# snphbaum/scikit-gpuppy

Hardware: AMD Instinct MI355X
Metric: GP fit+predict pts/sec (K+Cholesky, N=16384 d=8) (higher is better)
Workload: dtype f64; 1 GPU; C3: N=16384 d=8 M=16384 fit(Gram+Cholesky+alpha)+estimate_many, theta fixed; global_batch=32768, parallelism=1 GPU

## Files before the change

include/gpx.h:

```cpp
#ifndef GPX_H
#define GPX_H

#include <stdint.h>

#ifdef __cplusplus
extern "C" {
#endif

#define GPX_ABI_VERSION 1
#define GPX_MAX_D 64
#define GPX_TILE 128

#define GPX_ERR_BAD_ARG   (-1)
#define GPX_ERR_HIP       (-2)
#define GPX_ERR_NO_DEVICE (-3)
#define GPX_ERR_STATE     (-4)
#define GPX_INFO_STALLED  0x3fffffff

typedef struct gpx_handle gpx_handle;

int         gpx_abi_version(void);
const char *gpx_last_error(void);
int         gpx_device_count(void);
int         gpx_set_device(int device);
// ... 61 lines not shown
int gpx_spgp_fit(const double *x, const double *t_centered, int64_t n, int d, const double *theta, const double *xb,
                 int64_t m, gpx_spgp **out);
void gpx_spgp_free(gpx_spgp *h);
int gpx_spgp_predict(gpx_spgp *h, const double *xs, int64_t ms, double *mean , double *var );
int gpx_spgp_nll(gpx_spgp *h, double *nll);
int gpx_spgp_nll_grad(gpx_spgp *h, double *grad_out);
int gpx_spgp_dense(gpx_spgp *h, int which, double *out );
int gpx_spgp_cross(gpx_spgp *h, const double *xi, int64_t n1, const double *xj, int64_t n2, double *out );

enum {
    GPX_K_GRAM = 0,
    GPX_K_GEMM = 1,
    GPX_K_POTRF_LEAF = 2,
    GPX_K_TRSV = 3,
    GPX_K_REDUCE = 4,
    GPX_K_QUAD = 5,
    GPX_K_EXACT = 6,
    GPX_K_GEMM_SMALL = 7,
    GPX_K_TRSV_RIDE = 8,
    GPX_K_GEMM_EMU = 9,
    GPX_K_COUNT = 10
};
int gpx_profile_enable(gpx_handle *h, int level);
int gpx_profile_reset(gpx_handle *h);
int gpx_profile_read(gpx_handle *h, int kernel_class, int64_t *launches, double *total_ms, double *total_work);

int gpx_bench_mfma_f64(int iters, double *tflops);
int gpx_bench_emu_i8(int64_t rows, int64_t cols, int64_t K, int nmod, int iters, double *ms);
int gpx_emu_gemm_nt_sub(const double *A, int64_t lda, const double *B, int64_t ldb, double *C, int64_t ldc, int64_t rows, int64_t cols,
                        int64_t K);
int gpx_emu_rebuild(const int8_t *R, int64_t ldr, int64_t sr, int nmod, const int *sa, const int *sb, double *C, int64_t ldc, int64_t rows,
                    int64_t cols);
int gpx_emu_i8_gemm(const int8_t *A, const int8_t *B, int64_t rows, int64_t cols, int64_t K, int nmod, int8_t *R);
int gpx_emu_trsm_left(gpx_handle *h, double *Z, int64_t ldz, int64_t rows, const double *bound, double *Zs, int64_t tile_rows, int *status_out);
int gpx_bench_hbm(int64_t bytes, int iters, double *write_gbs, double *copy_gbs);
int gpx_bench_fp64_pipes(int blocks, int iters, int mode, double *tflops, double *cycles_per_inst, double *clock_ghz);

int gpx_dev_gram(const double *xi_dev, int64_t n1, const double *xj_dev, int64_t n2, int d, const double *theta,
                 double add_diag, int lower_only, int pad_identity,
                 double *out_dev, int64_t ld, int64_t rows_pad, int64_t cols_pad, void *stream);
int gpx_dev_gram_scaled(const double *xiw_dev, int64_t n1, const double *xjw_dev, int64_t n2, int d, double v, double add_diag,
                        int lower_only, int pad_identity, double *out_dev, int64_t ld, int64_t rows_pad, int64_t cols_pad,
                        void *stream);
int gpx_dev_gemm_nt(const double *A, int64_t lda, const double *B, int64_t ldb, double *C, int64_t ldc,
                    int64_t M, int64_t N, int64_t K, double alpha, double beta, int lower_only, void *stream);
int gpx_dev_syrk_trap(const double *A, int64_t lda, const double *B, int64_t ldb, double *C, int64_t ldc, int64_t M, int64_t off_cols,
                      int64_t K, double alpha, double beta, int *count_dev, void *stream);

enum {
    GPX_GEMM_TRI_NONE = 0,
    GPX_GEMM_TRI_A_UPPER = 1,
    GPX_GEMM_TRI_A_LOWER = 2,
    GPX_GEMM_TRI_B_LOWER = 3,
    GPX_GEMM_TRI_B_UPPER = 5
};
#define GPX_GEMM_VARIANT(wm, wn, lower, form) ((wm) | ((wn) << 4) | ((lower) << 8) | ((form) << 12))
enum { GPX_GEMM_FORM_NONE = 0, GPX_GEMM_FORM_FINE = 1, GPX_GEMM_FORM_LONGEST_FIRST = 2, GPX_GEMM_FORM_PAIRED = 3, GPX_GEMM_FORM_SMALL = 4 };
enum {
    GPX_GEMM_V_NONE = 0,
    GPX_GEMM_V_128X128 = GPX_GEMM_VARIANT(4, 4, 0, 0),
    GPX_GEMM_V_64X64 = GPX_GEMM_VARIANT(2, 2, 0, 0),
    GPX_GEMM_V_64X128 = GPX_GEMM_VARIANT(2, 4, 0, 0),
    GPX_GEMM_V_32X128 = GPX_GEMM_VARIANT(1, 4, 0, 0),
    GPX_GEMM_V_LOWER_128X128 = GPX_GEMM_VARIANT(4, 4, 1, 0),
    GPX_GEMM_V_LOWER_64X64 = GPX_GEMM_VARIANT(2, 2, 1, 0),
    GPX_GEMM_V_LOWER_32X32 = GPX_GEMM_VARIANT(1, 1, 1, 0),
// ... 46 lines not shown
```

scikit-gpuppy_amd/csrc/emu.hip:

```cpp
#include <math.h>
#include <stdint.h>
#include <stdlib.h>
#include <algorithm>

#include "common.h"

#include "gemm_tile.h"

typedef int v4i __attribute__((ext_vector_type(4)));
typedef int v16i __attribute__((ext_vector_type(16)));

constexpr int EMU_MAXL = 16;
constexpr int EMU_BT = 256;
constexpr int EMU_SLAB = 1024;
constexpr int EMU_BK = 128;

constexpr int EMU_MODULI[EMU_MAXL] = {256, 255, 253, 251, 247, 241, 239, 233, 229, 227, 223, 211, 199, 197, 193, 191};

static __constant__ const int emu_p[EMU_MAXL] = {256, 255, 253, 251, 247, 241, 239, 233, 229, 227, 223, 211, 199, 197, 193, 191};

typedef unsigned __int128 emu_u128;
struct EmuCrt {
    double m[EMU_MAXL][3], p[4], pinv;
    float c[EMU_MAXL];
    unsigned long p_lo, p_hi, half_lo, half_hi;
};
struct EmuCrtAll { EmuCrt t[EMU_MAXL + 1]; };
constexpr EmuCrtAll emu_crt_tables()
{
    EmuCrtAll all{};
    constexpr emu_u128 mask = ((emu_u128)1 << 40) - 1;
    for (int L = 2; L <= EMU_MAXL; ++L) {
        EmuCrt &t = all.t[L];
        emu_u128 P = 1;
        for (int l = 0; l < L; ++l) P *= (emu_u128)EMU_MODULI[l];
        for (int l = 0; l < L; ++l) {
            const emu_u128 M = P / (emu_u128)EMU_MODULI[l];
            const int p = EMU_MODULI[l], a = (int)(M % (emu_u128)p);
            int inv = 0;
            for (int x = 1; x < p; ++x)
                if (a * x % p == 1) { inv = x; break; }
            t.c[l] = (float)inv;
            for (int j = 0; j < 3; ++j) t.m[l][j] = (double)(unsigned long)((M >> (40 * j)) & mask);
// ... 8 lines not shown
    return all;
}
static constexpr EmuCrtAll emu_crt = emu_crt_tables();

#ifdef EMU_STAMP
constexpr int EMU_STAMP_SLOTS = 1 << 16;
__device__ unsigned long emu_stamps[EMU_STAMP_SLOTS][4];
extern "C" int gpx_emu_stamps(unsigned long *out, int n)
{
    return hipMemcpyFromSymbol(out, HIP_SYMBOL(emu_stamps), sizeof(unsigned long) * 4 * std::min(n, EMU_STAMP_SLOTS)) == hipSuccess ? 0 : GPX_ERR_HIP;
}
#endif

constexpr int EMU_NONFINITE = 0x7fffffff;

int emu_moduli()
{
    static const int v = [] { const char *e = getenv("GPX_EMU_MODULI"); const int l = e ? atoi(e) : EMU_MAXL; return std::min(EMU_MAXL, std::max(2, l)); }();
    return v;
}
bool emu_enabled(int64_t K)
{
    static const int on = [] { const char *e = getenv("GPX_EMU_F64"); return e ? atoi(e) : 1; }();
    static const long min_k = [] { const char *e = getenv("GPX_EMU_MIN_K"); return e ? atol(e) : 4096L; }();
    return on && K >= min_k && K < (1 << 17) && K % EMU_BK == 0;
}
int emu_scale_bits(int64_t K, int L)
{
    double log2p = 0.0;
    for (int l = 0; l < L; ++l) log2p += log2((double)EMU_MODULI[l]);
    return (int)floor(log2p - 1.0 - log2((double)K) - 1e-9);
}

static __device__ __forceinline__ void emu_store_residues(const double (&a)[4], int L, int8_t *__restrict__ out, long plane)
{
#pragma unroll
    for (int l = 0; l < EMU_MAXL; ++l) {
        if (l >= L) continue;
        const double p = (double)emu_p[l], pinv = 1.0 / p, h = 0.5 * p;
        unsigned packed = 0;
#pragma unroll
        for (int e = 0; e < 4; ++e) {
            double r = fma(-rint(a[e] * pinv), p, a[e]);
            r = r > h ? r - p : (r < -h ? r + p : r);
            packed |= ((unsigned)(int)r & 0xffu) << (8 * e);
        }
        *reinterpret_cast<unsigned *>(out + l * plane) = packed;
    }
}

__global__ __launch_bounds__(256) void emu_split_kernel(const double *__restrict__ X, long ldx, long rows_real, int K, int bits, int L,
                                                        int8_t *__restrict__ res, long plane, int *__restrict__ sig)
{
    const long row = blockIdx.x;
    const int t = threadIdx.x;
    __shared__ double red_max[4];
    __shared__ int red_bad[4];
    int8_t *out = res + row * (long)K;
    if (row >= rows_real) {
        for (int c = 4 * t; c < K; c += 1024)
            for (int l = 0; l < L; ++l) *reinterpret_cast<int *>(out + l * plane + c) = 0;
        if (t == 0) sig[row] = 0;
        return;
    }
    const double *x = X + row * ldx;
    double m = 0.0;
    int bad = 0;
    for (int c = 2 * t; c < K; c += 512) {
        const v2d v = *reinterpret_cast<const v2d *>(x + c);
        bad |= (int)!isfinite(v.x) | (int)!isfinite(v.y);
        m = fmax(m, fmax(fabs(v.x), fabs(v.y)));
    }
#pragma unroll
    for (int o = 32; o > 0; o >>= 1) { m = fmax(m, __shfl_xor(m, o)); bad |= __shfl_xor(bad, o); }
    if ((t & 63) == 0) { red_max[t >> 6] = m; red_bad[t >> 6] = bad; }
    __syncthreads();
    m = fmax(fmax(red_max[0], red_max[1]), fmax(red_max[2], red_max[3]));
    bad = red_bad[0] | red_bad[1] | red_bad[2] | red_bad[3];
    const int s = (bad || m == 0.0) ? 0 : bits - 1 - ilogb(m);
    if (t == 0) sig[row] = bad ? EMU_NONFINITE : s;
    for (int c = 4 * t; c < K; c += 1024) {
        const v2d v0 = *reinterpret_cast<const v2d *>(x + c), v1 = *reinterpret_cast<const v2d *>(x + c + 2);
        double a[4] = {rint(ldexp(v0.x, s)), rint(ldexp(v0.y, s)), rint(ldexp(v1.x, s)), rint(ldexp(v1.y, s))};
        if (bad) a[0] = a[1] = a[2] = a[3] = 0.0;
        emu_store_residues(a, L, out + c, plane);
    }
}

__global__ __launch_bounds__(256) void emu_split_fixed_kernel(const double *__restrict__ X, long ldx, long rows_real, int width, int bits, int L,
                                                              int8_t *__restrict__ res, long ldr, long plane, int *sig, int *status)
{
    const long row = blockIdx.x;
    const int t = threadIdx.x;
    int8_t *out = res + row * ldr;
    if (row >= rows_real) {
        for (int c = 4 * t; c < width; c += 1024)
            for (int l = 0; l < L; ++l) *reinterpret_cast<int *>(out + l * plane + c) = 0;
        return;
    }
    const double *x = X + row * ldx;
    const int s0 = sig[row];
    const bool dead = s0 == EMU_NONFINITE;
    const int s = dead ? 0 : s0;
    const double lim = ldexp(1.0, bits);
    int bad = 0, over = 0;
    for (int c = 4 * t; c < width; c += 1024) {
        const v2d v0 = *reinterpret_cast<const v2d *>(x + c), v1 = *reinterpret_cast<const v2d *>(x + c + 2);
        const double v[4] = {v0.x, v0.y, v1.x, v1.y};
        double a[4];
#pragma unroll
        for (int e = 0; e < 4; ++e) {
            a[e] = rint(ldexp(v[e], s));
            if (!isfinite(v[e])) { bad = 1; a[e] = 0.0; }
            else if (fabs(a[e]) > lim) { over = 1; a[e] = 0.0; }
            if (dead) a[e] = 0.0;
        }
        emu_store_residues(a, L, out + c, plane);
    }
    bad = __syncthreads_or(bad);
    over = __syncthreads_or(over);
    if (t == 0) {
        if (bad) sig[row] = EMU_NONFINITE;
        else if (over && !dead) atomicMax(status, 1);
    }
}

constexpr int EMU_ZERO_BOUND_SCALE = 1000;
__global__ __launch_bounds__(256) void emu_scale_from_bound_kernel(const double *__restrict__ bound, long rows, long rows_pad, int bits,
                                                                   int *__restrict__ sig, int *status)
{
    const long i = (long)blockIdx.x * 256 + threadIdx.x;
    if (i >= rows_pad) return;
    const double b = i < rows ? bound[i] : 0.0;
    int s = 0;
    if (!(b >= 0.0) || isinf(b)) atomicMax(status, 1);
    else s = b == 0.0 ? EMU_ZERO_BOUND_SCALE : bits - 2 - ilogb(b);
    sig[i] = s;
}

__global__ __launch_bounds__(512, 1) void emu_i8_gemm_kernel(const int8_t *__restrict__ A, const int8_t *__restrict__ B, long sa, long sb, int K,
                                                             int8_t *__restrict__ R, long ldr, long sr, int tm, int tn, int lda)
{
    __shared__ __attribute__((aligned(1024))) int8_t smem[2 * 2 * EMU_BT * EMU_BK];
    constexpr int STAGE = 2 * EMU_BT * EMU_BK;
    const int nwg = gridDim.x, orig = blockIdx.x;
    const int lid = xcd_chunk_start(nwg, orig & 7) + (orig >> 3);
    const int per = tm * tn, z = lid / per;
    int rem = lid - z * per;
    const int g = rem / (8 * tn), first = 8 * g, grows = std::min(8, tm - first);
    rem -= g * 8 * tn;
    const int bx = rem / grows, by = first + rem - bx * grows;

    const int t = threadIdx.x;
    const int wave = __builtin_amdgcn_readfirstlane(t >> 6), lane = t & 63;
    const int wr = wave >> 2, wc = wave & 3;
    const int drow = lane >> 3;
// ... 109 lines not shown
#pragma unroll
    for (int l = 0; l < EMU_MAXL; ++l)
        w[l] = l < L ? *reinterpret_cast<const unsigned *>(R + l * sr + i * ldr + j0) : 0u;
    const int si = sa[i];
    double *c = C + i * ldc + j0;
    const __int128 P = (__int128)(((emu_u128)T.p_hi << 64) | T.p_lo), half = (__int128)(((emu_u128)T.half_hi << 64) | T.half_lo);
#pragma unroll
    for (int e = 0; e < 4; ++e) {
        if (j0 + e >= cols) continue;
        const int tj = sb[j0 + e];
        if (si == EMU_NONFINITE || tj == EMU_NONFINITE) { c[e] = __builtin_nan(""); continue; }
        double s0 = 0.0, s1 = 0.0, s2 = 0.0;
#pragma unroll
        for (int l = 0; l < EMU_MAXL; ++l) {
            const float pl = (float)emu_p[l], plinv = 1.0f / pl;
            float t = (float)(int8_t)(w[l] >> (8 * e)) * T.c[l];
            t = fmaf(-rintf(t * plinv), pl, t);
            const double td = (double)t;
            s0 = fma(td, T.m[l][0], s0);
            s1 = fma(td, T.m[l][1], s1);
            s2 = fma(td, T.m[l][2], s2);
        }
        const double q = rint(fma(fma(s2, 0x1p40, s1), 0x1p40, s0) * T.pinv);
        const long x0 = (long)fma(-q, T.p[0], s0), x1 = (long)fma(-q, T.p[1], s1), x2 = (long)fma(-q, T.p[2], s2), x3 = (long)(-q * T.p[3]);
        __int128 X = (__int128)((emu_u128)(__int128)x0 + ((emu_u128)(__int128)x1 << 40) + ((emu_u128)(__int128)x2 << 80) + ((emu_u128)(__int128)x3 << 120));
        X = X >= half ? X - P : (X < -half ? X + P : X);
        const long hi = (long)(X >> 64);
        const unsigned long lo = (unsigned long)X;
        const double xd = (hi == ((long)lo >> 63)) ? (double)(long)lo : fma((double)hi, 0x1p64, (double)lo);
        c[e] -= ldexp(xd, -(si + tj));
    }
}

static int64_t emu_cap(int64_t K, int L) { return std::max<int64_t>(EMU_BT, (((int64_t)1 << 31) / (K * L)) / EMU_BT * EMU_BT); }

void emu_work_need(EmuWork &w, int64_t rows, int64_t cols, int64_t K)
{
    const int L = emu_moduli();
    const int64_t cap = emu_cap(K, L), rt = std::min(round_up(rows, EMU_BT), cap), ct = std::min(round_up(cols, EMU_BT), cap);
    w.a_bytes = std::max(w.a_bytes, rt * K * L);
    w.b_bytes = std::max(w.b_bytes, ct * K * L);
    w.r_bytes = std::max(w.r_bytes, std::min(rt * ct * L, (int64_t)1 << 31));
    w.sig_n = std::max(w.sig_n, rt + ct);
}

int emu_work_alloc(EmuWork &w, Scratch &sc)
{
    GPX_TRY(sc.take(&w.ra, w.a_bytes));
    GPX_TRY(sc.take(&w.rb, w.b_bytes));
    GPX_TRY(sc.take(&w.rr, w.r_bytes));
    return sc.take(&w.sig, w.sig_n);
}

static int emu_check_args(const double *A, int64_t lda, const double *B, int64_t ldb, int64_t ldc, int64_t cols, int64_t K)
{
    if (K <= 0 || K % EMU_BK || K >= (1 << 17)) {
        gpx_set_error("emu_gemm_nt_sub: K = %ld is not a multiple of %d in [%d, 2^17)", (long)K, EMU_BK, EMU_BK);
        return GPX_ERR_BAD_ARG;
    }
    if (lda < K || ldb < K || ldc < cols) {
        gpx_set_error("emu_gemm_nt_sub: leading dimension shorter than a row (lda %ld, ldb %ld < K %ld, or ldc %ld < cols %ld)", (long)lda, (long)ldb,
                      (long)K, (long)ldc, (long)cols);
        return GPX_ERR_BAD_ARG;
    }
    if ((lda | ldb) & 1 || ((uintptr_t)A | (uintptr_t)B) & 15) {
        gpx_set_error("emu_gemm_nt_sub: A and B must be 16-byte aligned with even lda, ldb (lda %ld, ldb %ld, A %p, B %p)", (long)lda, (long)ldb,
                      (const void *)A, (const void *)B);
        return GPX_ERR_BAD_ARG;
    }
    return 0;
}

int emu_gemm_nt_sub(const double *A, int64_t lda, const double *B, int64_t ldb, double *C, int64_t ldc, int64_t rows, int64_t cols, int64_t K,
                    const EmuWork &w, hipStream_t s, Profiler *prof)
{
    if (rows <= 0 || cols <= 0) return 0;
    if (K % EMU_BK || K >= (1 << 17)) { gpx_set_error("emu_gemm_nt_sub: K = %ld out of range", (long)K); return GPX_ERR_BAD_ARG; }
    const int L = emu_moduli();
    const int bits = emu_scale_bits(K, L), abits = bits - bits / 2, bbits = bits / 2;
    const int64_t cap = emu_cap(K, L);
    const int64_t rt = std::min<int64_t>(round_up(rows, EMU_BT), cap);
    int64_t ct = std::min<int64_t>(round_up(cols, EMU_BT), cap);
    while (ct > EMU_BT && rt * ct * L > ((int64_t)1 << 31)) ct -= EMU_BT;
    if (!w.ra || rt * K * L > w.a_bytes || ct * K * L > w.b_bytes || rt * ct * L > w.r_bytes || rt + ct > w.sig_n) {
        gpx_set_error("emu_gemm_nt_sub: workspace too small for %ld x %ld x %ld", (long)rows, (long)cols, (long)K);
        return GPX_ERR_STATE;
    }
    ProfScope ps(prof, s, GPX_K_GEMM_EMU, 2.0 * (double)rows * (double)cols * (double)K);
    int8_t *ra = w.ra, *rb = w.rb, *rr = w.rr;
    int *sga = w.sig, *sgb = sga + rt;
    for (int64_t r0 = 0; r0 < rows; r0 += rt) {
        const int64_t nr = std::min(rt, rows - r0), nrp = round_up(nr, EMU_BT);
        hipLaunchKernelGGL(emu_split_kernel, dim3((unsigned)nrp), dim3(256), 0, s, A + r0 * lda, (long)lda, (long)nr, (int)K, abits, L, ra,
                           (long)(nrp * K), sga);
        for (int64_t c0 = 0; c0 < cols; c0 += ct) {
            const int64_t nc = std::min(ct, cols - c0), ncp = round_up(nc, EMU_BT);
            hipLaunchKernelGGL(emu_split_kernel, dim3((unsigned)ncp), dim3(256), 0, s, B + c0 * ldb, (long)ldb, (long)nc, (int)K, bbits, L, rb,
                               (long)(ncp * K), sgb);
            const int tm = (int)(nrp / EMU_BT), tn = (int)(ncp / EMU_BT);
            hipLaunchKernelGGL(emu_i8_gemm_kernel, dim3((unsigned)(tm * tn * L)), dim3(512), 0, s, (const int8_t *)ra, (const int8_t *)rb,
                               (long)(nrp * K), (long)(ncp * K), (int)K, rr, (long)ncp, (long)(nrp * ncp), tm, tn, (int)K);
            const long thr = (long)nr * ((nc + 3) / 4);
            hipLaunchKernelGGL(emu_rebuild_kernel, dim3((unsigned)((thr + 255) / 256)), dim3(256), 0, s, (const int8_t *)rr, (long)ncp,
                               (long)(nrp * ncp), L, emu_crt.t[L], (const int *)sga, (const int *)sgb, C + r0 * ldc + c0, (long)ldc, (long)nr, (long)nc);
        }
        GPX_HIP(hipGetLastError());
    }
    return 0;
}

bool emu_left_enabled()
{
    static const int on = [] { const char *e = getenv("GPX_EMU_LEFT"); return e ? atoi(e) : 1; }();
    return on != 0;
}

bool emu_left_route(bool bounded, bool few, bool ready, int64_t slabs)
{
    return bounded && !few && ready && slabs >= 5 && emu_left_enabled() && emu_enabled(4 * EMU_SLAB);
}

void emu_left_plan(EmuLeft &w, int64_t rows, int64_t slabs, int64_t tile_rows)
{
    w.L = emu_moduli();
    w.lda = EMU_SLAB * (slabs - 1);
    const int bits = emu_scale_bits(w.lda, w.L);
    w.abits = bits - bits / 2;
    w.bbits = bits / 2;
    w.rows_pad = round_up(rows, EMU_BT);
    int64_t cap = emu_cap(w.lda, w.L);
    if (tile_rows > 0) cap = std::min(cap, round_up(tile_rows, EMU_BT));
// ... 5 lines not shown
}

int emu_left_alloc(EmuLeft &w, Scratch &sc)
{
    int rc = sc.take(&w.img, w.img_bytes);
    if (!rc) rc = sc.take(&w.rb, w.b_bytes);
    if (!rc) rc = sc.take(&w.rr, w.r_bytes);
    if (!rc) rc = sc.take(&w.sig, w.rows_pad + EMU_SLAB + 1);
    if (!rc) rc = sc.take(&w.bound, w.rows_pad);
    if (rc) {
        for (void *p : {(void *)w.img, (void *)w.rb, (void *)w.rr, (void *)w.sig, (void *)w.bound})
            if (p) dfree(sc.release((double *)p));
        w.img = w.rb = w.rr = nullptr;
        w.sig = nullptr;
        w.bound = nullptr;
    }
    return rc;
}

int emu_left_begin(const EmuLeft &w, const double *bound, int64_t rows, hipStream_t s)
{
    if (rows > w.rows_pad) { gpx_set_error("emu_left_begin: %ld rows in a workspace of %ld", (long)rows, (long)w.rows_pad); return GPX_ERR_STATE; }
    GPX_HIP(hipMemsetAsync(w.status(), 0, sizeof(int), s));
    hipLaunchKernelGGL(emu_scale_from_bound_kernel, dim3((unsigned)((w.rows_pad + 255) / 256)), dim3(256), 0, s, bound, (long)rows, (long)w.rows_pad,
                       w.abits, w.sig, w.status());
    GPX_HIP(hipGetLastError());
    return 0;
}

int emu_left_split(const EmuLeft &w, const double *X, int64_t ldx, int64_t rows, int64_t q, hipStream_t s)
{
    for (int64_t t = 0, r0 = 0; r0 < rows; ++t, r0 += w.rt) {
        const int64_t nr = std::min(w.rt, rows - r0), nrp = round_up(nr, EMU_BT);
        hipLaunchKernelGGL(emu_split_fixed_kernel, dim3((unsigned)nrp), dim3(256), 0, s, X + r0 * ldx, (long)ldx, (long)nr, EMU_SLAB, w.abits, w.L,
                           w.img + t * w.rt * w.lda * w.L + q * EMU_SLAB, (long)w.lda, (long)(w.rt * w.lda), w.sig + r0, w.status());
    }
    GPX_HIP(hipGetLastError());
    return 0;
}

int emu_left_update(const EmuLeft &w, const double *B, int64_t ldb, double *C, int64_t ldc, int64_t rows, int64_t cols, int64_t K, hipStream_t s,
                    Profiler *prof)
{
    if (K <= 0 || K > w.lda || K % EMU_SLAB || cols <= 0 || cols > EMU_SLAB || rows > w.rows_pad) {
        gpx_set_error("emu_left_update: %ld x %ld x %ld outside the image", (long)rows, (long)cols, (long)K);
        return GPX_ERR_STATE;
    }
    ProfScope ps(prof, s, GPX_K_GEMM_EMU, 2.0 * (double)rows * (double)cols * (double)K);
    const int64_t ncp = round_up(cols, EMU_BT);
    int *sgb = w.sig + w.rows_pad;
    hipLaunchKernelGGL(emu_split_kernel, dim3((unsigned)ncp), dim3(256), 0, s, B, (long)ldb, (long)cols, (int)K, w.bbits, w.L, w.rb, (long)(ncp * K), sgb);
    for (int64_t t = 0, r0 = 0; r0 < rows; ++t, r0 += w.rt) {
        const int64_t nr = std::min(w.rt, rows - r0), nrp = round_up(nr, EMU_BT);
        const int tm = (int)(nrp / EMU_BT), tn = (int)(ncp / EMU_BT);
        hipLaunchKernelGGL(emu_i8_gemm_kernel, dim3((unsigned)(tm * tn * w.L)), dim3(512), 0, s, (const int8_t *)(w.img + t * w.rt * w.lda * w.L),
                           (const int8_t *)w.rb, (long)(w.rt * w.lda), (long)(ncp * K), (int)K, w.rr, (long)ncp, (long)(nrp * ncp), tm, tn, (int)w.lda);
        const long thr = (long)nr * ((cols + 3) / 4);
        hipLaunchKernelGGL(emu_rebuild_kernel, dim3((unsigned)((thr + 255) / 256)), dim3(256), 0, s, (const int8_t *)w.rr, (long)ncp, (long)(nrp * ncp), w.L,
                           emu_crt.t[w.L], (const int *)(w.sig + r0), (const int *)sgb, C + r0 * ldc, (long)ldc, (long)nr, (long)cols);
    }
    GPX_HIP(hipGetLastError());
    return 0;
}

extern "C" int gpx_emu_gemm_nt_sub(const double *A, int64_t lda, const double *B, int64_t ldb, double *C, int64_t ldc, int64_t rows, int64_t cols,
                                   int64_t K)
{
    GPX_TRY(gpx_require_device());
    if (rows < 0 || cols < 0 || !A || !B || !C) { gpx_set_error("gpx_emu_gemm_nt_sub: bad arguments"); return GPX_ERR_BAD_ARG; }
    GPX_TRY(emu_check_args(A, lda, B, ldb, ldc, cols, K));
    if (rows == 0 || cols == 0) return 0;
    Scratch sc(0);
    EmuWork w;
    emu_work_need(w, rows, cols, K);
    GPX_TRY(emu_work_alloc(w, sc));
    int rc = emu_gemm_nt_sub(A, lda, B, ldb, C, ldc, rows, cols, K, w, 0, nullptr);
    if (hipStreamSynchronize(0) != hipSuccess && rc == 0) { gpx_set_error("gpx_emu_gemm_nt_sub: stream failed"); rc = GPX_ERR_HIP; }
    return rc;
}

extern "C" int gpx_emu_rebuild(const int8_t *R, int64_t ldr, int64_t sr, int nmod, const int *sa, const int *sb, double *C, int64_t ldc, int64_t rows,
                               int64_t cols)
{
    GPX_TRY(gpx_require_device());
    if (!R || !sa || !sb || !C || rows < 0 || cols < 0 || nmod < 2 || nmod > EMU_MAXL || ldr < round_up(cols, 4) || (ldr | sr) & 3 ||
        (uintptr_t)R & 3 || sr < rows * ldr || ldc < cols) {
        gpx_set_error("gpx_emu_rebuild: bad arguments");
        return GPX_ERR_BAD_ARG;
    }
    if (rows == 0 || cols == 0) return 0;
    const long thr = (long)rows * ((cols + 3) / 4);
    hipLaunchKernelGGL(emu_rebuild_kernel, dim3((unsigned)((thr + 255) / 256)), dim3(256), 0, 0, R, (long)ldr, (long)sr, nmod, emu_crt.t[nmod], sa, sb, C,
                       (long)ldc, (long)rows, (long)cols);
    GPX_HIP(hipGetLastError());
    GPX_HIP(hipStreamSynchronize(0));
    return 0;
}

extern "C" int gpx_emu_i8_gemm(const int8_t *A, const int8_t *B, int64_t rows, int64_t cols, int64_t K, int nmod, int8_t *R)
{
    GPX_TRY(gpx_require_device());
    if (!A || !B || !R || rows <= 0 || cols <= 0 || rows % EMU_BT || cols % EMU_BT || K <= 0 || K % EMU_BK || K >= (1 << 17) || nmod < 1 ||
        nmod > EMU_MAXL || ((uintptr_t)A | (uintptr_t)B) & 15 || rows / EMU_BT * (cols / EMU_BT) * nmod > INT32_MAX) {
        gpx_set_error("gpx_emu_i8_gemm: bad arguments");
        return GPX_ERR_BAD_ARG;
    }
    const int tm = (int)(rows / EMU_BT), tn = (int)(cols / EMU_BT);
    hipLaunchKernelGGL(emu_i8_gemm_kernel, dim3((unsigned)(tm * tn * nmod)), dim3(512), 0, 0, A, B, (long)(rows * K), (long)(cols * K), (int)K, R,
                       (long)cols, (long)(rows * cols), tm, tn, (int)K);
    GPX_HIP(hipGetLastError());
    GPX_HIP(hipStreamSynchronize(0));
    return 0;
}

__global__ void emu_fill_kernel(int8_t *p, long n, unsigned seed)
{
    for (long i = (long)blockIdx.x * 256 + threadIdx.x; i < n; i += (long)gridDim.x * 256) {
        unsigned x = (unsigned)i * 2654435761u ^ seed;
        x ^= x >> 15; x *= 2246822519u; x ^= x >> 13;
        p[i] = (int8_t)(x & 0xff);
    }
}

extern "C" int gpx_bench_emu_i8(int64_t rows, int64_t cols, int64_t K, int nmod, int iters, double *ms)
{
    GPX_TRY(gpx_require_device());
// ... 34 lines not shown
```

scikit-gpuppy_amd/skgpuppy_amd/_gpx.py:

```python
import ctypes
import os

import numpy as np

_HERE = os.path.dirname(os.path.abspath(__file__))
LIB_PATH = os.environ.get("GPX_LIB", os.path.join(_HERE, "libgpx.so"))

GPX_ERR_BAD_ARG, GPX_ERR_HIP, GPX_ERR_NO_DEVICE, GPX_ERR_STATE = -1, -2, -3, -4
K_GRAM, K_GEMM, K_POTRF_LEAF, K_TRSV, K_REDUCE, K_QUAD, K_EXACT, K_GEMM_SMALL, K_TRSV_RIDE, K_GEMM_EMU = range(10)
KERNEL_CLASS_NAMES = ["gram", "gemm_f64_mfma", "potrf_leaf", "trsv", "predict_reduce", "approx_quad", "exact_sum",
                      "gemm_f64_mfma_small_tiles", "trsv_under_factorisation", "gemm_f64_emulated_int8"]

GEMM_TRI_NONE, GEMM_TRI_A_UPPER, GEMM_TRI_A_LOWER, GEMM_TRI_B_LOWER, GEMM_TRI_B_UPPER = 0, 1, 2, 3, 5


def gemm_variant(wm, wn, lower, form):
    return wm | (wn << 4) | (lower << 8) | (form << 12)


GEMM_VARIANTS = {
    "NONE": 0,
    "128X128": gemm_variant(4, 4, 0, 0), "64X64": gemm_variant(2, 2, 0, 0), "64X128": gemm_variant(2, 4, 0, 0), "32X128": gemm_variant(1, 4, 0, 0),
    "LOWER_128X128": gemm_variant(4, 4, 1, 0), "LOWER_64X64": gemm_variant(2, 2, 1, 0), "LOWER_32X32": gemm_variant(1, 1, 1, 0),
    "TRIB_FINE": gemm_variant(2, 2, 0, 1), "TRIB_LONGEST_FIRST": gemm_variant(4, 4, 0, 2), "TRIB_PAIRED": gemm_variant(4, 4, 0, 3),
# ... 38 lines not shown
    "gpx_chol": (_int, [_hp, _dp]),
    "gpx_chol_rows": (_int, [_hp, _i64, _i64, _dp]),
    "gpx_kinv_rows": (_int, [_hp, _i64, _i64, _dp]),
    "gpx_cjh": (_int, [_hp, _dp, _dp, _dp, _dp]),
    "gpx_propagate_approx": (_int, [_hp, _dp, _dp] + [ctypes.POINTER(_dbl)] * 4),
    "gpx_propagate_approx_many": (_int, [_hp, _dp, _dp, _int, _i64, _dp, _dp, _dp, _dp]),
    "gpx_propagate_approx_rows": (_int, [_hp, _dp, _dp, _i64, _i64, _dp]),
    "gpx_propagate_approx_rhs": (_int, [_hp, _dp, _dp, _int, _int, _dp]),
    "gpx_propagate_dvh": (_int, [_hp, _dp, _dp]),
    "gpx_propagate_exact": (_int, [_hp, _dp, _dp, ctypes.POINTER(_dbl), ctypes.POINTER(_dbl)]),
    "gpx_propagate_exact_rows": (_int, [_hp, _dp, _dp, _i64, _i64, _dp]),
    "gpx_exact_mean": (_int, [_hp, _dp, _dp, ctypes.POINTER(_dbl)]),
    "gpx_propagate_exact_matrix": (_int, [_hp, _dp, _dp, _dp, _i64, _int, _dp, _dp, _dp, _dp, _dbl, ctypes.POINTER(_dbl), ctypes.POINTER(_dbl)]),
    "gpx_kinv_model_create": (_int, [_dp, _dp, _i64, ctypes.POINTER(_hp)]),
    "gpx_kinv_model_free": (None, [_hp]),
    "gpx_propagate_exact_model": (_int, [_hp, _dp, _int, _dp, _dp, _dp, _dp, _dbl, ctypes.POINTER(_dbl), ctypes.POINTER(_dbl)]),
    "gpx_nll": (_int, [_hp, ctypes.POINTER(_dbl)]),
    "gpx_nll_grad": (_int, [_hp, _dp]),
    "gpx_spgp_fit": (_int, [_dp, _dp, _i64, _int, _dp, _dp, _i64, ctypes.POINTER(_hp)]),
    "gpx_spgp_free": (None, [_hp]),
    "gpx_spgp_predict": (_int, [_hp, _dp, _i64, _dp, _dp]),
    "gpx_spgp_nll": (_int, [_hp, ctypes.POINTER(_dbl)]),
    "gpx_spgp_nll_grad": (_int, [_hp, _dp]),
    "gpx_spgp_dense": (_int, [_hp, _int, _dp]),
    "gpx_spgp_cross": (_int, [_hp, _dp, _i64, _dp, _i64, _dp]),
    "gpx_profile_enable": (_int, [_hp, _int]),
    "gpx_profile_reset": (_int, [_hp]),
    "gpx_profile_read": (_int, [_hp, _int, ctypes.POINTER(_i64), ctypes.POINTER(_dbl), ctypes.POINTER(_dbl)]),
    "gpx_bench_mfma_f64": (_int, [_int, ctypes.POINTER(_dbl)]),
    "gpx_bench_emu_i8": (_int, [_i64, _i64, _i64, _int, _int, ctypes.POINTER(_dbl)]),
    "gpx_emu_gemm_nt_sub": (_int, [_dp, _i64, _dp, _i64, _dp, _i64, _i64, _i64, _i64]),
    "gpx_emu_rebuild": (_int, [_dp, _i64, _i64, _int, _dp, _dp, _dp, _i64, _i64, _i64]),
    "gpx_emu_i8_gemm": (_int, [_dp, _dp, _i64, _i64, _i64, _int, _dp]),
    "gpx_emu_trsm_left": (_int, [_hp, _dp, _i64, _i64, _dp, _dp, _i64, ctypes.POINTER(_int)]),
    "gpx_bench_hbm": (_int, [_i64, _int, ctypes.POINTER(_dbl), ctypes.POINTER(_dbl)]),
    "gpx_bench_fp64_pipes": (_int, [_int, _int, _int] + [ctypes.POINTER(_dbl)] * 3),
    "gpx_dev_gram": (_int, [_dp, _i64, _dp, _i64, _int, _dp, _dbl, _int, _int, _dp, _i64, _i64, _i64, ctypes.c_void_p]),
    "gpx_dev_gram_scaled": (_int, [_dp, _i64, _dp, _i64, _int, _dbl, _dbl, _int, _int, _dp, _i64, _i64, _i64, ctypes.c_void_p]),
    "gpx_dev_gemm_nt": (_int, [_dp, _i64, _dp, _i64, _dp, _i64, _i64, _i64, _i64, _dbl, _dbl, _int, ctypes.c_void_p]),
    "gpx_dev_gemm_nt_ex": (_int, [_dp, _i64, _dp, _i64, _dp, _i64, _i64, _i64, _i64, _dbl, _dbl, _int, _int, _int, _int, ctypes.POINTER(_int),
                                  ctypes.c_void_p]),
    "gpx_dev_gemm_nt_tri_reduce": (_int, [_dp, _i64, _dp, _i64, _dp, _i64, _i64, _i64, _dbl, _dp, _dp, _dp, _i64, _i64, ctypes.c_void_p]),
    "gpx_dev_gemm_nt_batched": (_int, [_dp, _i64, _i64, _i64, _dp, _i64, _i64, _i64, _dp, _i64, _i64, _i64, _int, _int, _i64, _i64, _i64, _dbl,
                                       _dbl, _i64, ctypes.c_void_p]),
    "gpx_dev_syrk_splitk": (_int, [_dp, _i64, _dp, _dp, _i64, _i64, _int, _dbl, ctypes.c_void_p]),
    "gpx_dev_syrk_trap": (_int, [_dp, _i64, _dp, _i64, _dp, _i64, _i64, _i64, _i64, _dbl, _dbl, ctypes.c_void_p, ctypes.c_void_p]),
    "gpx_dev_potrf_leaf": (_int, [_dp, _i64, _dp, _dp, ctypes.c_void_p, _int, ctypes.c_void_p]),
    "gpx_dev_chol_panel": (_int, [_dp, _i64, _i64, _i64, _i64, _dp, _dp, ctypes.c_void_p, ctypes.c_void_p]),
    "gpx_dev_chol_panel_next": (_int, [_dp, _i64, _i64, _i64, _i64, _dp, _i64, _i64, _dp, _dp, ctypes.c_void_p, ctypes.c_void_p]),
    "gpx_dev_chol_panel_split": (_int, [_dp, _i64, _i64, _i64, _i64, _i64, _dp, _i64, _i64, _dp, _dp, ctypes.c_void_p, ctypes.c_void_p,
                                        ctypes.c_void_p, ctypes.c_void_p]),
    "gpx_dev_set_panel_share": (_int, [_int]),
    "gpx_dev_chol_dataflow": (_int, [_dp, _i64, _i64, _i64, _dp, _dp, ctypes.c_void_p, ctypes.c_void_p]),
    "gpx_adopt_factor": (_int, [_dp, _dp, _i64, _int, _dp, _dp, _dp, _dp, _dbl, ctypes.c_void_p, ctypes.POINTER(_hp)]),
    "gpx_multi_fit": (_int, [_dp, _dp, _i64, _int, _dp, ctypes.POINTER(_int), _int, ctypes.POINTER(_hp)]),
    "gpx_multi_free": (None, [_hp]),
    "gpx_multi_info": (_int, [_hp, ctypes.POINTER(_int), ctypes.POINTER(_i64), ctypes.POINTER(_dbl)]),
    "gpx_multi_alpha": (_int, [_hp, _dp]),
    "gpx_multi_predict": (_int, [_hp, _dp, _i64, _dp, _dp]),
    "gpx_multi_propagate_approx": (_int, [_hp, _dp, _dp] + [ctypes.POINTER(_dbl)] * 4),
    "gpx_multi_propagate_exact": (_int, [_hp, _dp, _dp] + [ctypes.POINTER(_dbl)] * 2),
}
for _name, (_res, _args) in SIGNATURES.items():
    try:
        _f = getattr(lib, _name)
    except AttributeError:
# ... 34 lines not shown
```

Before: 466,000 pts/s.

## Rewrite int8 residue split with integer dot4 reduction and wave-per-row layout

The f64-to-int8 residue split for the emulated FP64 GEMM is rebuilt. Each value is first split into two 32-bit words, then reduced modulo each small prime with udot4 against precomputed powers of 256 and a multiply-high reduction, replacing per-modulus double rint/fma. The row-scale computation moves into its own kernel, and the split now assigns 16 elements per lane with 128-bit stores, with the fixed split using one wave per row. Test entry points for both split kernels are also added. This cuts ALU work and gives wider stores in the preprocessing stage, at the cost of an extra launch and more intricate modular arithmetic.

```diff
diff --git a/include/gpx.h b/include/gpx.h
--- a/include/gpx.h
+++ b/include/gpx.h
@@ -117,6 +117,10 @@
 int gpx_emu_rebuild(const int8_t *R, int64_t ldr, int64_t sr, int nmod, const int *sa, const int *sb, double *C, int64_t ldc, int64_t rows,
                     int64_t cols);
 int gpx_emu_i8_gemm(const int8_t *A, const int8_t *B, int64_t rows, int64_t cols, int64_t K, int nmod, int8_t *R);
+int gpx_emu_split(const double *X, int64_t ldx, int64_t rows, int64_t rows_pad, int64_t K, int bits, int nmod, int8_t *res, int64_t plane,
+                  int *sig);
+int gpx_emu_split_fixed(const double *X, int64_t ldx, int64_t rows, int64_t rows_pad, int64_t width, int bits, int nmod, int8_t *res,
+                        int64_t ldr, int64_t plane, int *sig, int *status);
 int gpx_emu_trsm_left(gpx_handle *h, double *Z, int64_t ldz, int64_t rows, const double *bound, double *Zs, int64_t tile_rows, int *status_out);
 int gpx_bench_hbm(int64_t bytes, int iters, double *write_gbs, double *copy_gbs);
 int gpx_bench_fp64_pipes(int blocks, int iters, int mode, double *tflops, double *cycles_per_inst, double *clock_ghz);
diff --git a/scikit-gpuppy_amd/csrc/emu.hip b/scikit-gpuppy_amd/csrc/emu.hip
--- a/scikit-gpuppy_amd/csrc/emu.hip
+++ b/scikit-gpuppy_amd/csrc/emu.hip
@@ -9,6 +9,7 @@
 
 typedef int v4i __attribute__((ext_vector_type(4)));
 typedef int v16i __attribute__((ext_vector_type(16)));
+typedef unsigned v4u __attribute__((ext_vector_type(4)));
 
 constexpr int EMU_MAXL = 16;
 constexpr int EMU_BT = 256;
@@ -83,40 +84,113 @@
     return (int)floor(log2p - 1.0 - log2((double)K) - 1e-9);
 }
 
-static __device__ __forceinline__ void emu_store_residues(const double (&a)[4], int L, int8_t *__restrict__ out, long plane)
-{
-#pragma unroll
-    for (int l = 0; l < EMU_MAXL; ++l) {
-        if (l >= L) continue;
-        const double p = (double)emu_p[l], pinv = 1.0 / p, h = 0.5 * p;
-        unsigned packed = 0;
-#pragma unroll
-        for (int e = 0; e < 4; ++e) {
-            double r = fma(-rint(a[e] * pinv), p, a[e]);
-            r = r > h ? r - p : (r < -h ? r + p : r);
-            packed |= ((unsigned)(int)r & 0xffu) << (8 * e);
+struct EmuSplitMod { unsigned c0, c1, k0, m; };
+constexpr EmuSplitMod emu_split_mod(int l)
+{
+    const unsigned p = (unsigned)EMU_MODULI[l];
+    EmuSplitMod t{};
+    unsigned w = 1 % p;
+    for (int k = 0; k < 8; ++k) {
+        (k < 4 ? t.c0 : t.c1) |= w << (8 * (k & 3));
+        w = w * 256 % p;
+    }
+    unsigned b = 1 % p;
+    for (int i = 0; i < 60; ++i) b = 2 * b % p;
+    t.k0 = (p - b) % p;
+    t.m = (unsigned)((((unsigned long)1 << 31) + p - 1) / p);
+    return t;
+}
+static_assert(EMU_MODULI[0] == 256, "the first modulus takes the low byte as it is");
+
+static __device__ __forceinline__ void emu_words(double a, unsigned &lo, unsigned &hi)
+{
+    const double h = floor(a * 0x1p-32);
+    lo = (unsigned)fma(-h, 0x1p32, a);
+    hi = (unsigned)((int)h + (1 << 28));
+}
+
+template <int l> static __device__ __forceinline__ v4u emu_plane_bytes(const unsigned (&lo)[16], const unsigned (&hi)[16])
+{
+    int r[16];
+    if constexpr (l == 0) {
+#pragma unroll
+        for (int e = 0; e < 16; ++e) r[e] = (int)lo[e];
+    } else {
+        constexpr EmuSplitMod M = emu_split_mod(l);
+        constexpr int p = EMU_MODULI[l];
+        static_assert(p % 2 == 1 && p < 256 && M.m < (1u << 24), "the reduction below is for odd moduli of one byte");
+        unsigned x[16], q[16];
+#pragma unroll
+        for (int e = 0; e < 16; ++e) x[e] = __builtin_amdgcn_udot4(lo[e], M.c0, M.k0, false);
+#pragma unroll
+        for (int e = 0; e < 16; ++e) x[e] = __builtin_amdgcn_udot4(hi[e], M.c1, x[e], false);
+#pragma unroll
+        for (int e = 0; e < 16; ++e) q[e] = __umulhi((2u * x[e] + (unsigned)p) & 0xffffffu, M.m);
+#pragma unroll
+        for (int e = 0; e < 16; ++e) asm("v_mad_u32_u24 %0, %1, %2, %3" : "=v"(r[e]) : "v"(q[e]), "s"(256 - p), "v"(x[e]));
+    }
+    v4u out;
+#pragma unroll
+    for (int g = 0; g < 4; ++g) {
+        const unsigned w01 = __builtin_amdgcn_perm((unsigned)r[4 * g + 1], (unsigned)r[4 * g], 0x0c0c0400u);
+        const unsigned w23 = __builtin_amdgcn_perm((unsigned)r[4 * g + 3], (unsigned)r[4 * g + 2], 0x0c0c0400u);
+        out[g] = __builtin_amdgcn_perm(w23, w01, 0x05040100u);
+    }
+    return out;
+}
+
+template <int l> static __device__ __forceinline__ void emu_store_planes(const unsigned (&lo)[16], const unsigned (&hi)[16], int L,
+                                                                         int8_t *__restrict__ out, long plane)
+{
+    if constexpr (l < EMU_MAXL) {
+        if (l >= L) return;
+        *reinterpret_cast<v4u *>(out) = emu_plane_bytes<l>(lo, hi);
+        emu_store_planes<l + 1>(lo, hi, L, out + plane, plane);
+    }
+}
+
+template <bool CHECKED>
+static __device__ __forceinline__ void emu_split_lane(const double *__restrict__ x, bool zero, int s, double lim, int L, int8_t *__restrict__ out,
+                                                      long plane, int &bad, int &over)
+{
+    if (zero) {
+        for (int l = 0; l < L; ++l, out += plane) *reinterpret_cast<v4u *>(out) = (v4u){0u, 0u, 0u, 0u};
+        return;
+    }
+    v2d v[8];
+#pragma unroll
+    for (int j = 0; j < 8; ++j) v[j] = *reinterpret_cast<const v2d *>(x + 2 * j);
+    unsigned lo[16], hi[16];
+#pragma unroll
+    for (int e = 0; e < 16; ++e) {
+        const double xe = (e & 1) ? v[e >> 1].y : v[e >> 1].x;
+        double a = rint(ldexp(xe, s));
+        if (CHECKED) {
+            const bool nf = !isfinite(xe), ok = fabs(a) <= lim;
+            bad |= (int)nf;
+            over |= (int)(!ok && !nf);
+            a = ok ? a : 0.0;
         }
-        *reinterpret_cast<unsigned *>(out + l * plane) = packed;
-    }
-}
-
-__global__ __launch_bounds__(256) void emu_split_kernel(const double *__restrict__ X, long ldx, long rows_real, int K, int bits, int L,
-                                                        int8_t *__restrict__ res, long plane, int *__restrict__ sig)
+        emu_words(a, lo[e], hi[e]);
+    }
+    emu_store_planes<0>(lo, hi, L, out, plane);
+}
+
+__global__ __launch_bounds__(256) void emu_row_scale_kernel(const double *__restrict__ X, long ldx, long rows_real, int K, int bits,
+                                                            int *__restrict__ sig)
 {
     const long row = blockIdx.x;
     const int t = threadIdx.x;
+    if (row >= rows_real) {
+        if (t == 0) sig[row] = 0;
+        return;
+    }
     __shared__ double red_max[4];
     __shared__ int red_bad[4];
-    int8_t *out = res + row * (long)K;
-    if (row >= rows_real) {
-        for (int c = 4 * t; c < K; c += 1024)
-            for (int l = 0; l < L; ++l) *reinterpret_cast<int *>(out + l * plane + c) = 0;
-        if (t == 0) sig[row] = 0;
-        return;
-    }
     const double *x = X + row * ldx;
     double m = 0.0;
     int bad = 0;
+#pragma unroll 4
     for (int c = 2 * t; c < K; c += 512) {
         const v2d v = *reinterpret_cast<const v2d *>(x + c);
         bad |= (int)!isfinite(v.x) | (int)!isfinite(v.y);
@@ -126,53 +200,42 @@
     for (int o = 32; o > 0; o >>= 1) { m = fmax(m, __shfl_xor(m, o)); bad |= __shfl_xor(bad, o); }
     if ((t & 63) == 0) { red_max[t >> 6] = m; red_bad[t >> 6] = bad; }
     __syncthreads();
-    m = fmax(fmax(red_max[0], red_max[1]), fmax(red_max[2], red_max[3]));
-    bad = red_bad[0] | red_bad[1] | red_bad[2] | red_bad[3];
-    const int s = (bad || m == 0.0) ? 0 : bits - 1 - ilogb(m);
-    if (t == 0) sig[row] = bad ? EMU_NONFINITE : s;
-    for (int c = 4 * t; c < K; c += 1024) {
-        const v2d v0 = *reinterpret_cast<const v2d *>(x + c), v1 = *reinterpret_cast<const v2d *>(x + c + 2);
-        double a[4] = {rint(ldexp(v0.x, s)), rint(ldexp(v0.y, s)), rint(ldexp(v1.x, s)), rint(ldexp(v1.y, s))};
-        if (bad) a[0] = a[1] = a[2] = a[3] = 0.0;
-        emu_store_residues(a, L, out + c, plane);
-    }
-}
-
-__global__ __launch_bounds__(256) void emu_split_fixed_kernel(const double *__restrict__ X, long ldx, long rows_real, int width, int bits, int L,
-                                                              int8_t *__restrict__ res, long ldr, long plane, int *sig, int *status)
-{
-    const long row = blockIdx.x;
-    const int t = threadIdx.x;
-    int8_t *out = res + row * ldr;
-    if (row >= rows_real) {
-        for (int c = 4 * t; c < width; c += 1024)
-            for (int l = 0; l < L; ++l) *reinterpret_cast<int *>(out + l * plane + c) = 0;
-        return;
-    }
-    const double *x = X + row * ldx;
-    const int s0 = sig[row];
-    const bool dead = s0 == EMU_NONFINITE;
-    const int s = dead ? 0 : s0;
-    const double lim = ldexp(1.0, bits);
+    if (t == 0) {
+        m = fmax(fmax(red_max[0], red_max[1]), fmax(red_max[2], red_max[3]));
+        bad = red_bad[0] | red_bad[1] | red_bad[2] | red_bad[3];
+        sig[row] = bad ? EMU_NONFINITE : (m == 0.0 ? 0 : bits - 1 - ilogb(m));
+    }
+}
+
+__global__ __launch_bounds__(256) void emu_split_kernel(const double *__restrict__ X, long ldx, long rows_real, long rows_pad, int K, int L,
+                                                        int8_t *__restrict__ res, long plane, const int *__restrict__ sig)
+{
+    const int stretches = (K + 1023) >> 10;
+    const long item = (long)blockIdx.x * 4 + (threadIdx.x >> 6);
+    const long row = item / stretches;
+    const int c = (int)(item - row * stretches) * 1024 + 16 * (threadIdx.x & 63);
+    if (row >= rows_pad || c >= K) return;
+    const int s = row < rows_real ? sig[row] : EMU_NONFINITE;
     int bad = 0, over = 0;
-    for (int c = 4 * t; c < width; c += 1024) {
-        const v2d v0 = *reinterpret_cast<const v2d *>(x + c), v1 = *reinterpret_cast<const v2d *>(x + c + 2);
-        const double v[4] = {v0.x, v0.y, v1.x, v1.y};
-        double a[4];
-#pragma unroll
-        for (int e = 0; e < 4; ++e) {
-            a[e] = rint(ldexp(v[e], s));
-            if (!isfinite(v[e])) { bad = 1; a[e] = 0.0; }
-            else if (fabs(a[e]) > lim) { over = 1; a[e] = 0.0; }
-            if (dead) a[e] = 0.0;
-        }
-        emu_store_residues(a, L, out + c, plane);
-    }
-    bad = __syncthreads_or(bad);
-    over = __syncthreads_or(over);
-    if (t == 0) {
+    emu_split_lane<false>(X + row * ldx + c, s == EMU_NONFINITE, s, 0.0, L, res + row * (long)K + c, plane, bad, over);
+}
+
+__global__ __launch_bounds__(256) void emu_split_fixed_kernel(const double *__restrict__ X, long ldx, long rows_real, long rows_pad, int width,
+                                                              int bits, int L, int8_t *__restrict__ res, long ldr, long plane, int *sig, int *status)
+{
+    const long row = (long)blockIdx.x * 4 + (threadIdx.x >> 6);
+    const int lane = threadIdx.x & 63, c = 16 * lane;
+    if (row >= rows_pad) return;
+    const int s = row < rows_real ? sig[row] : EMU_NONFINITE;
+    const bool dead = s == EMU_NONFINITE;
+    int bad = 0, over = 0;
+    if (c < width) emu_split_lane<true>(X + row * ldx + c, dead, s, ldexp(1.0, bits), L, res + row * ldr + c, plane, bad, over);
+    if (dead) return;
+    bad = __any(bad);
+    over = __any(over);
+    if (lane == 0) {
         if (bad) sig[row] = EMU_NONFINITE;
-        else if (over && !dead) atomicMax(status, 1);
+        else if (over) atomicMax(status, 1);
     }
 }
 
@@ -348,6 +411,20 @@
     }
 }
 
+static void emu_launch_split(const double *X, long ldx, long rows, long rows_pad, int K, int bits, int L, int8_t *res, long plane, int *sig,
+                             hipStream_t s)
+{
+    const long waves = rows_pad * ((K + 1023) / 1024);
+    hipLaunchKernelGGL(emu_row_scale_kernel, dim3((unsigned)rows_pad), dim3(256), 0, s, X, ldx, rows, K, bits, sig);
+    hipLaunchKernelGGL(emu_split_kernel, dim3((unsigned)((waves + 3) / 4)), dim3(256), 0, s, X, ldx, rows, rows_pad, K, L, res, plane, (const int *)sig);
+}
+static void emu_launch_split_fixed(const double *X, long ldx, long rows, long rows_pad, int width, int bits, int L, int8_t *res, long ldr, long plane,
+                                   int *sig, int *status, hipStream_t s)
+{
+    hipLaunchKernelGGL(emu_split_fixed_kernel, dim3((unsigned)((rows_pad + 3) / 4)), dim3(256), 0, s, X, ldx, rows, rows_pad, width, bits, L, res, ldr,
+                       plane, sig, status);
+}
+
 static int64_t emu_cap(int64_t K, int L) { return std::max<int64_t>(EMU_BT, (((int64_t)1 << 31) / (K * L)) / EMU_BT * EMU_BT); }
 
 void emu_work_need(EmuWork &w, int64_t rows, int64_t cols, int64_t K)
@@ -407,12 +484,10 @@
     int *sga = w.sig, *sgb = sga + rt;
     for (int64_t r0 = 0; r0 < rows; r0 += rt) {
         const int64_t nr = std::min(rt, rows - r0), nrp = round_up(nr, EMU_BT);
-        hipLaunchKernelGGL(emu_split_kernel, dim3((unsigned)nrp), dim3(256), 0, s, A + r0 * lda, (long)lda, (long)nr, (int)K, abits, L, ra,
-                           (long)(nrp * K), sga);
+        emu_launch_split(A + r0 * lda, (long)lda, (long)nr, (long)nrp, (int)K, abits, L, ra, (long)(nrp * K), sga, s);
         for (int64_t c0 = 0; c0 < cols; c0 += ct) {
             const int64_t nc = std::min(ct, cols - c0), ncp = round_up(nc, EMU_BT);
-            hipLaunchKernelGGL(emu_split_kernel, dim3((unsigned)ncp), dim3(256), 0, s, B + c0 * ldb, (long)ldb, (long)nc, (int)K, bbits, L, rb,
-                               (long)(ncp * K), sgb);
+            emu_launch_split(B + c0 * ldb, (long)ldb, (long)nc, (long)ncp, (int)K, bbits, L, rb, (long)(ncp * K), sgb, s);
             const int tm = (int)(nrp / EMU_BT), tn = (int)(ncp / EMU_BT);
             hipLaunchKernelGGL(emu_i8_gemm_kernel, dim3((unsigned)(tm * tn * L)), dim3(512), 0, s, (const int8_t *)ra, (const int8_t *)rb,
                                (long)(nrp * K), (long)(ncp * K), (int)K, rr, (long)ncp, (long)(nrp * ncp), tm, tn, (int)K);
@@ -484,8 +559,8 @@
 {
     for (int64_t t = 0, r0 = 0; r0 < rows; ++t, r0 += w.rt) {
         const int64_t nr = std::min(w.rt, rows - r0), nrp = round_up(nr, EMU_BT);
-        hipLaunchKernelGGL(emu_split_fixed_kernel, dim3((unsigned)nrp), dim3(256), 0, s, X + r0 * ldx, (long)ldx, (long)nr, EMU_SLAB, w.abits, w.L,
-                           w.img + t * w.rt * w.lda * w.L + q * EMU_SLAB, (long)w.lda, (long)(w.rt * w.lda), w.sig + r0, w.status());
+        emu_launch_split_fixed(X + r0 * ldx, (long)ldx, (long)nr, (long)nrp, EMU_SLAB, w.abits, w.L, w.img + t * w.rt * w.lda * w.L + q * EMU_SLAB,
+                               (long)w.lda, (long)(w.rt * w.lda), w.sig + r0, w.status(), s);
     }
     GPX_HIP(hipGetLastError());
     return 0;
@@ -501,7 +576,7 @@
     ProfScope ps(prof, s, GPX_K_GEMM_EMU, 2.0 * (double)rows * (double)cols * (double)K);
     const int64_t ncp = round_up(cols, EMU_BT);
     int *sgb = w.sig + w.rows_pad;
-    hipLaunchKernelGGL(emu_split_kernel, dim3((unsigned)ncp), dim3(256), 0, s, B, (long)ldb, (long)cols, (int)K, w.bbits, w.L, w.rb, (long)(ncp * K), sgb);
+    emu_launch_split(B, (long)ldb, (long)cols, (long)ncp, (int)K, w.bbits, w.L, w.rb, (long)(ncp * K), sgb, s);
     for (int64_t t = 0, r0 = 0; r0 < rows; ++t, r0 += w.rt) {
         const int64_t nr = std::min(w.rt, rows - r0), nrp = round_up(nr, EMU_BT);
         const int tm = (int)(nrp / EMU_BT), tn = (int)(ncp / EMU_BT);
@@ -544,6 +619,44 @@
     const long thr = (long)rows * ((cols + 3) / 4);
     hipLaunchKernelGGL(emu_rebuild_kernel, dim3((unsigned)((thr + 255) / 256)), dim3(256), 0, 0, R, (long)ldr, (long)sr, nmod, emu_crt.t[nmod], sa, sb, C,
                        (long)ldc, (long)rows, (long)cols);
+    GPX_HIP(hipGetLastError());
+    GPX_HIP(hipStreamSynchronize(0));
+    return 0;
+}
+
+static bool emu_split_args_ok(const double *X, int64_t ldx, int64_t rows, int64_t rows_pad, int64_t width, int bits, int nmod, const int8_t *res,
+                              int64_t ldr, int64_t plane, const int *sig)
+{
+    return X && res && sig && rows >= 0 && rows <= rows_pad && rows_pad < ((int64_t)1 << 31) && width > 0 && bits >= 1 && bits <= 59 && nmod >= 1 &&
+           nmod <= EMU_MAXL && ldx >= width && !(ldx & 1) && !((uintptr_t)X & 15) && !((uintptr_t)res & 15) && ldr >= width && !(ldr & 15) &&
+           !(plane & 15) && plane >= (rows_pad - 1) * ldr + width;
+}
+
+extern "C" int gpx_emu_split(const double *X, int64_t ldx, int64_t rows, int64_t rows_pad, int64_t K, int bits, int nmod, int8_t *res, int64_t plane,
+                             int *sig)
+{
+    GPX_TRY(gpx_require_device());
+    if (K % EMU_BK || K >= (1 << 17) || !emu_split_args_ok(X, ldx, rows, rows_pad, K, bits, nmod, res, K, plane, sig)) {
+        gpx_set_error("gpx_emu_split: bad arguments");
+        return GPX_ERR_BAD_ARG;
+    }
+    if (rows_pad == 0) return 0;
+    emu_launch_split(X, (long)ldx, (long)rows, (long)rows_pad, (int)K, bits, nmod, res, (long)plane, sig, 0);
+    GPX_HIP(hipGetLastError());
+    GPX_HIP(hipStreamSynchronize(0));
+    return 0;
+}
+
+extern "C" int gpx_emu_split_fixed(const double *X, int64_t ldx, int64_t rows, int64_t rows_pad, int64_t width, int bits, int nmod, int8_t *res,
+                                   int64_t ldr, int64_t plane, int *sig, int *status)
+{
+    GPX_TRY(gpx_require_device());
+    if (!status || width % 16 || width > EMU_SLAB || !emu_split_args_ok(X, ldx, rows, rows_pad, width, bits, nmod, res, ldr, plane, sig)) {
+        gpx_set_error("gpx_emu_split_fixed: bad arguments");
+        return GPX_ERR_BAD_ARG;
+    }
+    if (rows_pad == 0) return 0;
+    emu_launch_split_fixed(X, (long)ldx, (long)rows, (long)rows_pad, (int)width, bits, nmod, res, (long)ldr, (long)plane, sig, status, 0);
     GPX_HIP(hipGetLastError());
     GPX_HIP(hipStreamSynchronize(0));
     return 0;
diff --git a/scikit-gpuppy_amd/skgpuppy_amd/_gpx.py b/scikit-gpuppy_amd/skgpuppy_amd/_gpx.py
--- a/scikit-gpuppy_amd/skgpuppy_amd/_gpx.py
+++ b/scikit-gpuppy_amd/skgpuppy_amd/_gpx.py
@@ -94,6 +94,8 @@
     "gpx_emu_gemm_nt_sub": (_int, [_dp, _i64, _dp, _i64, _dp, _i64, _i64, _i64, _i64]),
     "gpx_emu_rebuild": (_int, [_dp, _i64, _i64, _int, _dp, _dp, _dp, _i64, _i64, _i64]),
     "gpx_emu_i8_gemm": (_int, [_dp, _dp, _i64, _i64, _i64, _int, _dp]),
+    "gpx_emu_split": (_int, [_dp, _i64, _i64, _i64, _i64, _int, _int, _dp, _i64, _dp]),
+    "gpx_emu_split_fixed": (_int, [_dp, _i64, _i64, _i64, _i64, _int, _int, _dp, _i64, _i64, _dp, _dp]),
     "gpx_emu_trsm_left": (_int, [_hp, _dp, _i64, _i64, _dp, _dp, _i64, ctypes.POINTER(_int)]),
     "gpx_bench_hbm": (_int, [_i64, _int, ctypes.POINTER(_dbl), ctypes.POINTER(_dbl)]),
     "gpx_bench_fp64_pipes": (_int, [_int, _int, _int] + [ctypes.POINTER(_dbl)] * 3),
```

Result: faster. 475,500 pts/s, median of 6 (+2.0%).
